# riveSunder/therldaisyworld

Measured on AMD Instinct MI355X. Metric: cell-updates/sec (grid x batch), fused stencil+growth step, higher is better.
Workload: dtype f32

## Files before the change

therldaisyworld_amd/csrc/dw_api.hip:

```cpp
#include <hip/hip_runtime.h>

#include <cmath>
#include <cstdarg>
#include <cstdio>
#include <cstdlib>
#include <cstring>
#include <memory>
#include <new>
#include <type_traits>
#include <vector>

#include "../../include/daisyworld_hip.h"
#include "dw_kernels.hpp"
#include "dw_host_util.hpp"
#include "dw_plan.hpp"
#include "dw_series.hpp"

using namespace dw;

static thread_local char g_err[512] = "";

static int fail(int code, const char* fmt, ...) {
    va_list ap;
    va_start(ap, fmt);
// ... 436 lines not shown
        });
    } else {
        const int prec = p.precision == DW_PRECISION_F64 ? 2 : (ex ? 0 : 1);
        with_int<2, 0, 1>(prec, [&](auto PR) { generic(iL, iD, PR); });
    }
    HIPCHK(hipGetLastError());
    step_done(h, 0.0, true, true, constants);
    return DW_OK;
}

static int launch_forward_fused2_pw(dw_handle* h, const PairPw* row, StatsDev* trace) {
    const StepPlan& pl = h->plan;
    const StepOut o = step_out(h);
    const FusedGeom& g = pl.fgeom;
    const dim3 grid((unsigned)g.chunk * 8u);
    const plane_t *inL = h->L16[h->cur].get(), *inD = h->D16[h->cur].get();
    with_int<kFusedRot, kFusedOvl>(pl.fused_mode, [&](auto MODE) {
        hipLaunchKernelGGL((trace_pair_fast_pw<MODE>), grid, dim3(256), 0, h->stream, inL, inD, o.L, o.D, g, row, o.zero_me,
                           o.zero_n, trace);
    });
    HIPCHK(hipGetLastError());
    step_done(h, 0.0, false, true, true);
    return DW_OK;
}

static int temp_chunks(const dw_handle* h) {
    return (int)(((long long)h->prm.height * h->prm.width + kTempChunk - 1) / kTempChunk);
}
static size_t temp_part_bytes(const dw_handle* h) { return sizeof(TempPartial) * (size_t)h->prm.batch * temp_chunks(h); }

static int launch_temp_moments(dw_handle* h, bool current, double L, const PhysF64* row64, TempStatsDev* out) {
    const dw_params& p = h->prm;
    const int chunks = temp_chunks(h);
    const PhysF64 P = row64 ? PhysF64{} : make_f64(p, L);
    TempPartial* part = h->temp_part.get();
    auto reduce = [&](auto* iL, auto* iD) {
        with_bool(row64 != nullptr, [&](auto TABLE) {
            hipLaunchKernelGGL((temp_moments_pw<elem_t<decltype(iL)>, TABLE>), dim3((unsigned)chunks, (unsigned)p.batch), dim3(256),
                               0, h->stream, iL, iD, p.height, p.width, P, row64, part);
        });
    };
    if (current) with_planes(h, h->unq == OWN_CUR, h->cur, reduce);
    else with_derived_from(h, [&](auto* iL, auto* iD, auto) { reduce(iL, iD); });
    HIPCHK(hipGetLastError());
    hipLaunchKernelGGL(temp_moments_finish_pw, dim3((unsigned)((p.batch + 63) / 64)), dim3(64), 0, h->stream, part, p.batch, chunks,
                       (double)p.height * (double)p.width, out);
    HIPCHK(hipGetLastError());
    return DW_OK;
}

template <class F>
static auto with_fused_layout(const StepPlan& pl, F&& f) {
    if (pl.packed) return f(int_c<kFusedRot>{}, std::true_type{});
    return with_int<kFusedRot, kFusedRing, kFusedOvl>(pl.fused_mode, [&](auto MODE) { return f(MODE, std::false_type{}); });
}

static int launch_forward_fused2(dw_handle* h, double L1, double L2, unsigned int* pstats = nullptr,
                                 float thr_hi = 0.f, StatsDev* trace = nullptr) {
    const dw_params& p = h->prm;
    const StepPlan& pl = h->plan;
    const bool exact = p.precision == DW_PRECISION_EXACT;
    PhysF32 P1, P2;
    if (exact) derive_f32_pair(p, L1, L2, &P1, &P2);
    else { P1 = derive_f32(p, L1); P2 = derive_f32(p, L2); }
    const StepOut o = step_out(h);
    const FusedGeom& g = pl.fgeom;
    const dim3 grid((unsigned)g.chunk * 8u);
    const plane_t *inL = h->L16[h->cur].get(), *inD = h->D16[h->cur].get();
    auto exact_args = [&] {
        return FusedExactArgs{inL, inD, o.L, o.D, g, P1, lum_part(P2), o.zero_me, o.zero_n, pstats, thr_hi, make_f64(p, L1), L1, L2};
    };
    if (trace && exact) {
        const TraceExactArgs A{exact_args(), trace, h->sw.force_rescan ? 1 : 0};
        with_int<kFusedRot, kFusedOvl>(pl.fused_mode, [&](auto MODE) {
            with_bool(pl.sym_albedo, [&](auto SYM) {
                hipLaunchKernelGGL((trace_pair_exact<MODE, SYM>), grid, dim3(256), 0, h->stream, A);
            });
        });
    } else if (trace) {
        with_int<kFusedRot, kFusedOvl>(pl.fused_mode, [&](auto MODE) {
            hipLaunchKernelGGL((trace_pair_fast<MODE>), grid, dim3(256), 0, h->stream, inL, inD, o.L, o.D, g, P1, P2, o.zero_me,
                               o.zero_n, trace);
        });
    } else if (pl.fmt_planes && !pstats && !exact) {
        hipLaunchKernelGGL((step_stream_fused2_fmt_pw<kFusedOvl>), grid, dim3(256), 0, h->stream, inL, inD, o.L, o.D, g, P1, P2,
                           o.zero_me, o.zero_n);
    } else if (exact) {
        const FusedExactArgs A = exact_args();
        with_bool(pstats != nullptr, [&](auto STATS) {
            with_fused_layout(pl, [&](auto MODE, auto PACK) {
                with_bool(pl.sym_albedo, [&](auto SYM) {
                    hipLaunchKernelGGL((step_stream_fused2_exact<MODE, PACK, STATS, SYM>), grid, dim3(256), 0, h->stream, A);
                });
            });
        });
    } else {
        with_bool(pstats != nullptr, [&](auto STATS) {
            with_fused_layout(pl, [&](auto MODE, auto PACK) {
                hipLaunchKernelGGL((step_stream_fused2<MODE, PACK, STATS>), grid, dim3(256), 0, h->stream, inL, inD, o.L, o.D, g,
                                   P1, P2, o.zero_me, o.zero_n, pstats, thr_hi);
            });
        });
    }
    HIPCHK(hipGetLastError());
    step_done(h, L2, false);
    return DW_OK;
}

static int launch_agents(dw_handle* h, const int* d_action, int act_b, int act_n, bool standalone = false,
                         double* d_reward = nullptr, unsigned char* d_done = nullptr, unsigned char* d_ok = nullptr) {
    const dw_params& p = h->prm;
    if (p.n_agents == 0) return DW_OK;
    NEED(h->have_state, DW_ESTATE, "no state uploaded");
    NEED(h->have_agents, DW_ESTATE, "no agents uploaded (call dw_upload_agents or dw_init_random)");
    NEED(p.collision_mode == 0 || standalone, DW_EINVAL,
         "collision_mode=1: call dw_update_agents, apply the collision pass (it consumes the caller's RNG) to the "
         "downloaded agent states, upload them, then dw_step without actions");
    const int blocks = (p.batch + 63) / 64;
    with_planes(h, h->unq == OWN_CUR, h->cur, [&](auto* L, auto* D) {
        using T = elem_t<decltype(L)>;
        hipLaunchKernelGGL(agents_update<T>, dim3(blocks), dim3(64), 0, h->stream, L, D, h->idx.get(), h->st.get(), d_action,
                           act_b, act_n, p.batch, p.n_agents, p.height, p.width, p.agent_gamma,
                           p.collision_mode == 0 ? 1 : 0, d_reward, d_done, d_ok);
    });
    HIPCHK(hipGetLastError());
    return DW_OK;
}

static int stage_host_actions(dw_handle* h, const int32_t* action, int b, int n) {
    const dw_params& p = h->prm;
    NEED(b >= 0 && n >= 0 && b <= p.batch && n <= p.n_agents, DW_EINVAL,
         "action block %dx%d exceeds (B,N)=(%d,%d)", b, n, p.batch, p.n_agents);
    if ((size_t)b * n)
        HIPCHK(hipMemcpyAsync(h->action_tmp.get(), action, sizeof(int) * (size_t)b * n, hipMemcpyHostToDevice,
                              h->stream));
    return DW_OK;
}

static int clear_stats(dw_handle* h) {
    for (int i = 0; i < 2; ++i) HIPCHK(hipMemsetAsync(h->stats2[i].get(), 0, h->stats_bytes, h->stream));
    return DW_OK;
}

static void state_arrived(dw_handle* h, UnqOwner unq, UnqKind kind = UNQ_F64) {
    if (unq == OWN_CUR) h->unq_kind = kind;
    h->unq = unq;
    h->have_state = true;
    h->stepped = false;
    for (auto& sn : h->snap) sn.valid = false;
}

template <class T>
static auto init_random_into(dw_handle* h, uint64_t seed, T* L, T* D) {
    const dw_params& p = h->prm;
    if (int crc = clear_stats(h)) return crc;
    const int ncell = p.height * p.width;
    const dim3 g((unsigned)((ncell + kInitChunk - 1) / kInitChunk), (unsigned)p.batch);
    hipLaunchKernelGGL((init_random_cells<T>), g, dim3(256), 0, h->stream, L, D, ncell,
                       (long long)p.world_offset, (unsigned long long)seed, (float)p.light_proportion,
                       (float)p.dark_proportion, (float)p.initial_al, (float)p.initial_ad, h->stats2[h->sp].get());
    HIPCHK(hipGetLastError());
    if (p.n_agents) {
        const int bn = p.batch * p.n_agents;
        hipLaunchKernelGGL(init_random_agents, dim3((bn + 255) / 256), dim3(256), 0, h->stream, h->idx.get(), h->st.get(),
                           p.batch, p.n_agents, p.height, p.width, (long long)p.world_offset,
                           (unsigned long long)seed);
// ... 1555 lines not shown
        job(h->idx.get(), sn.idx.get(), sizeof(int) * 2 * bn);
        job(h->st.get(), sn.st.get(), sizeof(double) * bn);
    }
    if (sn.stepped && sn.unq != OWN_PREV) {
        job(h->L16[1 - h->cur].get(), sn.PL.get(), pb);
        job(h->D16[1 - h->cur].get(), sn.PD.get(), pb);
    }
    if (int rc = launch_copy_regions(h, J)) return rc;
    HIPCHK(hipMemsetAsync(h->stats2[1 - h->sp].get(), 0, h->stats_bytes, h->stream));
    h->unq = sn.unq;
    h->stepped = sn.stepped;
    h->L_last = sn.L_last;
    h->L_per_world = sn.L_per_world;
    h->P_per_world = sn.P_per_world;
    return DW_OK;
}

int dw_snapshot_save(dw_handle* h) { return dw_snapshot_save_slot(h, 0); }
int dw_snapshot_restore(dw_handle* h) { return dw_snapshot_restore_slot(h, 0); }


int dw_set_stream(dw_handle* h, void* hip_stream) {
    NEED(h, DW_EINVAL, "null handle");
    HIPCHK(hipSetDevice(h->prm.device));
    HIPCHK(hipStreamSynchronize(h->stream));
    if (h->own_stream) HIPCHK(hipStreamDestroy(h->stream));
    h->stream = reinterpret_cast<hipStream_t>(hip_stream);
    h->own_stream = false;
    return DW_OK;
}

int dw_sync(dw_handle* h) {
    NEED(h, DW_EINVAL, "null handle");
    HIPCHK(hipSetDevice(h->prm.device));
    HIPCHK(hipStreamSynchronize(h->stream));
    return DW_OK;
}

int dw_timer_start(dw_handle* h) {
    NEED(h, DW_EINVAL, "null handle");
    HIPCHK(hipSetDevice(h->prm.device));
    HIPCHK(hipEventRecord(h->ev0, h->stream));
    return DW_OK;
}

int dw_timer_stop(dw_handle* h, float* elapsed_ms) {
    NEED(h && elapsed_ms, DW_EINVAL, "null argument");
    HIPCHK(hipSetDevice(h->prm.device));
    HIPCHK(hipEventRecord(h->ev1, h->stream));
    HIPCHK(hipEventSynchronize(h->ev1));
    HIPCHK(hipEventElapsedTime(elapsed_ms, h->ev0, h->ev1));
    return DW_OK;
}

int dw_device_planes(dw_handle* h, int which, void** light, void** dark) {
    NEED(h && light && dark, DW_EINVAL, "null argument");
    NEED(which == DW_STATE_CURRENT || which == DW_STATE_PREVIOUS, DW_EINVAL, "bad state selector");
    const int buf = which == DW_STATE_CURRENT ? h->cur : 1 - h->cur;
    NEED(which != DW_STATE_CURRENT || cur_quantised(h), DW_ESTATE,
         "the current state is an un-quantised upload: it has no binary16 planes before the first step");
    *light = h->L16[buf].get();
    *dark = h->D16[buf].get();
    return DW_OK;
}

int dw_kernel_info(dw_handle* h, char* buf, size_t buflen) {
    NEED(h && buf && buflen, DW_EINVAL, "null argument");
    const dw_params& p = h->prm;
    const StepPlan& pl = h->plan;
    const char* prec = p.precision == DW_PRECISION_EXACT ? "exact" : (p.precision == DW_PRECISION_FAST ? "fast" : "f64");
    static const char* const halo_name[] = {"rotate", "dpp-old", "general", "packed"};
    if (pl.kind == STEP_STREAM) {
        const StripGeom& g = pl.sgeom;
        snprintf(buf, buflen,
                 "step_stream_%s<halo=%s> wave-strip=%dx256 cells, register window + DPP neighbours, %d-row blocks in "
                 "flight%s, %d strips, grid=%d x 256 threads (4 strips each), XCD-chunked",
                 prec, halo_name[pl.halo], g.SR,
                 p.precision == DW_PRECISION_EXACT ? DW_STREAM_RB_EXACT : DW_STREAM_RB_FAST,
                 p.precision == DW_PRECISION_EXACT ? ", in-wave float64 fix-up from an LDS queue" : "", g.nstrips,
                 g.chunk * 8);
        if (pl.allow_fuse) {
            const size_t n = std::strlen(buf);
            snprintf(buf + n, buflen - n, "; dw_step_n fuses step pairs (step_stream_fused2%s%s)",
                     p.precision == DW_PRECISION_EXACT ? "_exact" : "", pl.fmt_planes ? "_fmt_pw, format buffer accesses" : "");
        }
    } else if (pl.kind == STEP_TILED) {
        const int TR = (256 / pl.tcq) * pl.rpt;
        snprintf(buf, buflen,
                 "step_tiled<TCQ=%d,RPT=%d,%s> tile=%dx%d cells, %zu B LDS/workgroup, %d tiles, grid=%d x 256 threads, "
                 "XCD-chunked",
                 pl.tcq, pl.rpt, prec, TR, pl.tcq * 4, pl.tile_lds, pl.geom.ntiles, pl.geom.chunk * 8);
    } else {
        snprintf(buf, buflen, "step_generic<%s> one thread per cell, grid=(%d,%d) x 256 threads", prec,
                 (p.height * p.width + 255) / 256, p.batch);
    }
    {
        const size_t n = std::strlen(buf);
        snprintf(buf + n, buflen - n, pl.trace_pairs ? "; trace: step pairs" : "; trace: single steps");
    }
    {
        const size_t n = std::strlen(buf);
        snprintf(buf + n, buflen - n, pl.pw_stream ? "; per-world L: wave strips" : "; per-world L: generic");
    }
    {
        static const char* const form_name[] = {"launches per step", "workgroup (LDS)", "one wave per world"};
        const size_t n = std::strlen(buf);
        snprintf(buf + n, buflen - n, "; episode: %s; mlp episode: %s", form_name[episode_form(h)], form_name[episode_mlp_form(h)]);
    }
    {
        const size_t n = std::strlen(buf);
        snprintf(buf + n, buflen - n, "; ensemble episode: %s", ensemble_episode_wave(h) ? "one wave per world" : "launches per step");
    }
    if (pl.first_stream) {
        const size_t n = std::strlen(buf);
        snprintf(buf + n, buflen - n, "; first step: wave-strip=%dx256", pl.first_geom.SR);
    }
    if (h->sw.text[0]) {
        const size_t n = std::strlen(buf);
        snprintf(buf + n, buflen - n, "; switches[%s]", h->sw.text);
    }
    {
        const size_t n = std::strlen(buf);
        snprintf(buf + n, buflen - n, "; per-world constants: %s",
                 ensemble_pairs(h) ? "step pairs" : (pl.pw_stream ? "wave strips" : "generic"));
    }
    return DW_OK;
}

int dw_audit_tie_bound(dw_handle* h, double L, double out[4]) {
    NEED(h && out, DW_EINVAL, "null argument");
    const dw_params& p = h->prm;
    HIPCHK(hipSetDevice(p.device));
    NEED(h->have_state && cur_quantised(h), DW_ESTATE, "the audit needs a quantised current state");
    const StepPlan& pl = h->plan;
    int rc = ensure_scratch(h, 4 * sizeof(unsigned long long));
    if (rc) return rc;
    unsigned long long* d = reinterpret_cast<unsigned long long*>(h->scratch.get());
    HIPCHK(hipMemsetAsync(d, 0, 4 * sizeof(unsigned long long), h->stream));
    const dim3 g((unsigned)((p.height * p.width + 255) / 256), (unsigned)p.batch);
    hipLaunchKernelGGL(tie_audit, g, dim3(256), 0, h->stream, h->L16[h->cur].get(), h->D16[h->cur].get(), p.height, p.width,
                       derive_f32(p, L), make_f64(p, L), d, pl.sym_albedo && pl.kind == STEP_STREAM ? 1 : 0);
    HIPCHK(hipGetLastError());
    unsigned long long r[4];
    HIPCHK(hipMemcpyAsync(r, d, sizeof(r), hipMemcpyDeviceToHost, h->stream));
    HIPCHK(hipStreamSynchronize(h->stream));
    std::memcpy(&out[0], &r[0], sizeof(double));
    std::memcpy(&out[1], &r[1], sizeof(double));
    out[2] = (double)r[2];
    out[3] = (double)r[3];
    return DW_OK;
}

int dw_last_fixup_count(dw_handle* h, uint64_t* count) {
    NEED(h && count, DW_EINVAL, "null argument");
    HIPCHK(hipSetDevice(h->prm.device));
    std::vector<StatsDev> st((size_t)h->prm.batch + 1);
    HIPCHK(hipMemcpyAsync(st.data(), h->stats2[h->sp].get(), sizeof(StatsDev) * st.size(), hipMemcpyDeviceToHost, h->stream));
    HIPCHK(hipStreamSynchronize(h->stream));
    unsigned long long v = st[h->prm.batch].sum_l;
    for (int b = 0; b < h->prm.batch; ++b) v += st[b].reserved;
    *count = v;
    return DW_OK;
}

}
```

therldaisyworld_amd/csrc/dw_kernels.hpp:

```cpp
#pragma once
#include "dw_common.hpp"
#include "dw_step_generic.hpp"
#include "dw_step_tiled.hpp"
#include "dw_step_stream.hpp"
#include "dw_step_fused.hpp"
#include "dw_step_first.hpp"
#include "dw_step_per_world.hpp"
#include "dw_step_fused_pw.hpp"
#include "dw_episode.hpp"
#include "dw_episode_wave.hpp"
#include "dw_agents.hpp"
#include "dw_state_io.hpp"
#include "dw_agents_fused.hpp"
#include "dw_temp_moments.hpp"
#include "dw_episode_wave_pw.hpp"
```

therldaisyworld_amd/csrc/dw_plan.hpp:

```cpp
#pragma once
#include <climits>
#include <cmath>
#include <cstddef>
#include <cstdio>
#include <cstdlib>
#include <cstring>

#include "../../include/daisyworld_hip.h"
#include "dw_types.hpp"

namespace dw {

struct Switches {
    bool no_sym = false, no_pack = false, no_fuse = false, no_ring = false, no_fmt_planes = false, no_episode_kernel = false,
         no_episode_wave = false, no_agent_fuse = false, no_agent_preapply = false, first_f64 = false,
         first_generic = false, force_rescan = false, test_hooks = false;
    int pack_min_strips = -1, strip_rows = 0, tile_rpt = 0, queue_cap = -1, mismatch_cap = -1, trace_rows = 0;
    double first_slack = -1.0;
    char kernel[16] = {0};
    char text[256] = {0};
};
inline const char* test_hook(const char* name) {
    return std::getenv("DW_TEST_HOOKS") ? std::getenv(name) : nullptr;
}
inline Switches read_switches() {
    Switches w;
    auto note = [&](const char* name, const char* val) {
        const size_t n = std::strlen(w.text);
        snprintf(w.text + n, sizeof(w.text) - n, "%s%s%s%s", n ? " " : "", name, val ? "=" : "", val ? val : "");
    };
    auto flag = [&](const char* name, bool& dst) { if (std::getenv(name)) { dst = true; note(name, nullptr); } };
    auto num = [&](const char* name, int& dst, bool test) {
        if (const char* e = test ? test_hook(name) : std::getenv(name)) { dst = std::atoi(e); note(name, e); }
    };
    w.test_hooks = std::getenv("DW_TEST_HOOKS") != nullptr;
    flag("DW_NO_SYM", w.no_sym); flag("DW_NO_PACK", w.no_pack); flag("DW_NO_FUSE", w.no_fuse); flag("DW_NO_RING", w.no_ring);
    flag("DW_NO_FMT_PLANES", w.no_fmt_planes);
    flag("DW_NO_EPISODE_KERNEL", w.no_episode_kernel); flag("DW_NO_EPISODE_WAVE", w.no_episode_wave);
    flag("DW_NO_AGENT_FUSE", w.no_agent_fuse); flag("DW_NO_AGENT_PREAPPLY", w.no_agent_preapply);
    flag("DW_FIRST_STEP_F64", w.first_f64); flag("DW_FIRST_GENERIC", w.first_generic);
    num("DW_PACK_MIN_STRIPS", w.pack_min_strips, false); num("DW_STRIP_ROWS", w.strip_rows, false);
    num("DW_TILE_RPT", w.tile_rpt, false);
    num("DW_TEST_QUEUE_CAP", w.queue_cap, true); num("DW_TEST_MISMATCH_CAP", w.mismatch_cap, true);
    num("DW_TEST_TRACE_ROWS", w.trace_rows, true);
    if (test_hook("DW_TEST_FORCE_RESCAN")) { w.force_rescan = true; note("DW_TEST_FORCE_RESCAN", nullptr); }
    if (const char* e = test_hook("DW_TEST_FIRST_SLACK")) { w.first_slack = std::atof(e); note("DW_TEST_FIRST_SLACK", e); }
    if (const char* e = std::getenv("DW_KERNEL")) { snprintf(w.kernel, sizeof(w.kernel), "%s", e); note("DW_KERNEL", e); }
    return w;
}

inline dw_params with_world_params(dw_params p, const dw_world_params& w) {
    p.p = w.p; p.g = w.g; p.S = w.S; p.sigma = w.sigma; p.gamma = w.gamma; p.q = w.q; p.q2 = w.q2; p.dt = w.dt;
    p.albedo_bare = w.albedo_bare; p.albedo_light = w.albedo_light; p.albedo_dark = w.albedo_dark;
    p.temp_optimal = w.temp_optimal;
    return p;
}
inline dw_world_params world_params_of(const dw_params& p) {
    return dw_world_params{p.p, p.g, p.S, p.sigma, p.gamma, p.q, p.q2, p.dt, p.albedo_bare, p.albedo_light, p.albedo_dark,
                           p.temp_optimal};
}
inline bool albedo_symmetric(double bare, double light, double dark) { return (dark - bare) == -(light - bare); }
inline bool worlds_symmetric(const dw_world_params* worlds, size_t B) {
    for (size_t b = 0; b < B; ++b)
        if (!albedo_symmetric(worlds[b].albedo_bare, worlds[b].albedo_light, worlds[b].albedo_dark)) return false;
    return true;
}

inline PhysF64 make_f64(const dw_params& p, double L) {
    PhysF64 P;
    P.p = p.p; P.g = p.g; P.S = p.S; P.sigma = p.sigma; P.gamma = p.gamma; P.q = p.q; P.q2 = p.q2;
    P.dt = p.dt; P.ab = p.albedo_bare; P.al = p.albedo_light; P.ad = p.albedo_dark;
    P.To = p.temp_optimal; P.L = L;
    const double e1 = std::exp(-1.0), e2 = std::exp(-2.0);
    const double s = 1.0 + 4.0 * e1 + 4.0 * e2;
    P.w0 = 1.0 / s; P.w1 = e1 / s; P.w2 = e2 / s;
    return P;
}

inline double cbeta_host(const dw_params& p) {
    const double cbeta = p.g * p.temp_optimal * p.temp_optimal;
    return cbeta > 1e-30 ? 1.0 / std::sqrt(cbeta) : 0x1p60;
}

inline void split_hi_lo(double v, double scale, float* hi, float* lo) {
    const double h = std::nearbyint(v * scale) / scale;
    *hi = (float)h;
    *lo = (float)(v - h);
}

inline float round_up(double v) {
    const float f = (float)v;
    return (double)f < v ? std::nextafterf(f, INFINITY) : f;
}

struct EConst { double c0l, c0d; };
inline EConst e_const(const dw_params& p, double L) {
    const double To4 = std::pow(p.temp_optimal, 4), K = p.S * L / p.sigma;
    const double e0 = K * (1.0 - p.albedo_bare * p.p) / To4 - 1.0;
    return EConst{e0 + p.q2 * (p.albedo_bare * p.p - p.albedo_light) / To4,
                  e0 + p.q2 * (p.albedo_bare * p.p - p.albedo_dark) / To4};
}

struct TieChain {
    double emin, emax, vlo;
    bool admissible;
    double ew;
    double kbmax;
    double pu, safety;
};
inline TieChain tie_chain(const dw_params& p, const EConst& c, double a1, double a2, double a3, double a4, double de) {
    const double u = std::ldexp(1.0, -24), kmax = 1000.0;
    TieChain t;
    const double pos = (std::fmax(a1, 0.0) + std::fmax(a2, 0.0)) * 8 * kmax + (std::fmax(a3, 0.0) + std::fmax(a4, 0.0)) * kmax;
    const double neg = (std::fmin(a1, 0.0) + std::fmin(a2, 0.0)) * 8 * kmax + (std::fmin(a3, 0.0) + std::fmin(a4, 0.0)) * kmax;
    t.emax = std::fmax(c.c0l, c.c0d) + pos;
    t.emin = std::fmin(c.c0l, c.c0d) + neg;
    const double vmin = 1.0 + t.emin, vmax = 1.0 + t.emax;
    t.admissible = vmin > 0.02;
    t.vlo = std::fmax(vmin, 0.02);
    const double smax = std::sqrt(std::fmax(vmax, t.vlo));
// ... 39 lines not shown
    P.a1 = (float)((double)P.a1h + P.a1l); P.a2 = (float)((double)P.a2h + P.a2l);
    P.a3 = (float)((double)P.a3h + P.a3l); P.a4 = (float)((double)P.a4h + P.a4l);
    P.c0ls = (float)((double)P.c0lh + P.c0ll); P.c0ds = (float)((double)P.c0dh + c0dl);
    const double kbe = cbeta_host(p);
    P.kbeta = (float)kbe;
    const PhysF64 P64 = make_f64(p, L);
    P.dw0 = (float)(p.dt * P64.w0); P.dw1 = (float)(p.dt * P64.w1); P.dw2 = (float)(p.dt * P64.w2);
    P.p = (float)p.p; P.ck = p.dt != 0.0 ? (float)(0.001 / p.dt) : 0.f;
    P.ngamma = (float)(-p.gamma);
    const double u = std::ldexp(1.0, -24);
    const double lo_mag = std::ldexp(1.0, -(hb + 1)) * 18.0 * kmax + std::ldexp(1.0, -(hb + 1));
    const double de_abs = 6.0 * u * lo_mag + 1e-9;
    const TieChain t = tie_chain(p, c0, a1, a2, a3, a4, de_abs);
    auto e_over_D2 = [&](double e) {
        const double v = std::fmax(1.0 + e, t.vlo), sv = std::sqrt(v), yv = std::sqrt(sv);
        const double D = kbe * (yv + 1.0) * (sv + 1.0);
        return std::fabs(e) / (D * D);
    };
    const double Ae = 2.0 * de_abs * std::fmax(e_over_D2(t.emin), e_over_D2(t.emax));
    double A0 = t.safety * (kmax * std::fabs(p.dt) * t.kbmax * Ae + 2e-6);
    if (!t.admissible) A0 = 1.0;
    const double eA = t.safety * 13.0 * u;
    const double eK0d = t.safety * (6.0 * std::fabs(p.p) + t.pu + t.kbmax + 8.0 * std::fabs(p.gamma)) * u;
    const double eK1d = t.safety * ((6.0 * std::fabs(p.p) + t.pu) * u + t.kbmax * (u + 2.0 * t.ew));
    P.tie_lo = (float)(0.5 - A0);
    if ((double)P.tie_lo > 0.5 - A0) P.tie_lo = std::nextafterf(P.tie_lo, -INFINITY);
    P.eA = round_up(eA);
    const float eK0 = round_up(eK0d), eK1 = round_up(eK1d);
    P.eK0s = p.dt < 0.0 ? eK0 : -eK0;
    P.eK1s = p.dt < 0.0 ? eK1 : -eK1;
    P.neK1s = -P.eK1s;
    P.eK01s = (float)((double)P.eK0s + (double)P.eK1s);
    if (std::fabs((double)P.eK01s) < std::fabs((double)P.eK0s + (double)P.eK1s))
        P.eK01s = std::nextafterf(P.eK01s, P.eK01s < 0.f ? -1.f : 1.f);
    return P;
}

inline void derive_f32_pair(const dw_params& p, double L1, double L2, PhysF32* P1, PhysF32* P2) {
    const PhysF32 a = derive_f32(p, L1), b = derive_f32(p, L2);
    const int hb = a.hi_bits < b.hi_bits ? a.hi_bits : b.hi_bits;
    *P1 = derive_f32(p, L1, hb);
    *P2 = derive_f32(p, L2, hb);
    const float tie_lo = P1->tie_lo < P2->tie_lo ? P1->tie_lo : P2->tie_lo;
    P1->tie_lo = tie_lo;
    P2->tie_lo = tie_lo;
}

inline FirstStepBound derive_first_bound(const dw_params& p, double L, const PhysF32& P, bool from_f64,
                                         double test_slack = -1.0) {
    const double u = std::ldexp(1.0, -24), iota = from_f64 ? u : 0.0;
    const double kmax = 1000.0;
    const double a1 = std::fabs((double)P.a1), a2 = std::fabs((double)P.a2), a3 = std::fabs((double)P.a3), a4 = std::fabs((double)P.a4);
    const EConst c0 = e_const(p, L);
    const double c0m = std::fmax(std::fabs(c0.c0l), std::fabs(c0.c0d));
    const double Mmax = (a1 + a2) * 8 * kmax + (a3 + a4) * kmax;
    const double de_max = (8.0 * u + iota) * Mmax + u * c0m;
    const TieChain t = tie_chain(p, c0, P.a1, P.a2, P.a3, P.a4, de_max);
    const double kbe = cbeta_host(p);
    const double Dmin = kbe * (std::sqrt(std::sqrt(t.vlo)) + 1.0) * (std::sqrt(t.vlo) + 1.0);
    const double kK = 5.0 * u + iota;
    const double safety = t.safety, pu = t.pu, kbmax = t.kbmax;
    FirstStepBound B;
    B.a1 = round_up(a1); B.a2 = round_up(a2); B.a3 = round_up(a3); B.a4 = round_up(a4);
    B.c_de = round_up(safety * (8.0 * u + iota) * (1.0 + 8.0 * u));
    B.c_c0 = round_up(safety * u * c0m);
    B.eK0 = round_up(safety * (pu + (kK + 2.0 * u) * std::fabs(p.p) + kbmax * u + ((kK + 3.0 * u) + u) * std::fabs(p.gamma)));
    B.eK1 = round_up(safety * (pu + (kK + 2.0 * u) * std::fabs(p.p) + kbmax * (u + 2.0 * t.ew)));
    B.cW = round_up(safety * 2.0 * kbmax / Dmin);
    B.eA = round_up(safety * ((kK + 3.0 * u) + u + (kK + u)));
    B.cS = round_up(safety * u);
    B.slack = t.admissible ? 4e-6f : 1.0f;
    if (test_slack > (double)B.slack) B.slack = (float)test_slack;
    return B;
}

enum StepKind { STEP_GENERIC, STEP_TILED, STEP_STREAM };
struct StepPlan {
    StepKind kind = STEP_GENERIC;
    int halo = 0;
    bool packed = false;
    bool allow_fuse = false;
    int fused_mode = kFusedOvl;
    bool fmt_planes = false;
    bool trace_pairs = false;
    bool sym_albedo = false;
    int tcq = 0, rpt = 0;
    Geom geom{};
    size_t tile_lds = 0;
    StripGeom sgeom{};
    FusedGeom fgeom{};
    int first_prec = 2;
    bool first_stream = false;
    FirstGeom first_geom{};
    bool need_fixq = false;
    bool pw_stream = false;
};

inline int halo_form(int W) { return W < 256 ? 3 : (W == 256 ? 0 : (W % 256 == 0 ? 1 : 2)); }

inline int strip_rows(long groups, int H, long target) {
    int sr = 64;
    while (sr > 8 && groups * ((H + sr - 1) / sr) < target) sr >>= 1;
    return H < sr ? H : sr;
}

inline int strip_rows_or_override(const Switches& sw, int cap, long groups, int H, long target) {
    if (sw.strip_rows < 1) return strip_rows(groups, H, target);
    const int want = sw.strip_rows < cap ? sw.strip_rows : cap;
    return H < want ? H : want;
}

inline StepPlan plan_steps(const dw_params& p, const Switches& sw) {
    StepPlan s;
    s.sym_albedo = albedo_symmetric(p.albedo_bare, p.albedo_light, p.albedo_dark) && !sw.no_sym;
    s.halo = halo_form(p.width);
    const int lpw = p.width / 4, wpr = lpw ? 64 / lpw : 0;
    const bool pack_shape = p.width >= 8 && p.width < 256 && wpr >= 1 && wpr * lpw * 10 >= 64 * 7 && !sw.no_pack;
    const long pack_strips = pack_shape ? (long)((p.batch + wpr - 1) / wpr) * ((p.height + 63) / 64) : 0;
    const bool packable = pack_shape && pack_strips >= (sw.pack_min_strips >= 0 ? sw.pack_min_strips : 512);
    const bool quads = p.precision != DW_PRECISION_F64 && p.width % 4 == 0;
    if (quads && (p.width >= 256 || packable) && std::strcmp(sw.kernel, "tiled") != 0) {
        s.kind = STEP_STREAM;
        s.packed = p.width < 256;
        StripGeom& g = s.sgeom;
        g.B = p.batch; g.H = p.height; g.W = p.width;
        g.ncs = (p.width + 255) / 256;
        g.lpw = s.packed ? lpw : 64;
        g.wpr = s.packed ? wpr : 1;
        const long groups = s.packed ? (p.batch + wpr - 1) / wpr : p.batch;
        g.SR = strip_rows_or_override(sw, INT_MAX, groups * g.ncs, p.height, 2048);
        g.nrs = (p.height + g.SR - 1) / g.SR;
        g.nstrips = (int)(groups * g.nrs * g.ncs);
        g.nwg = (g.nstrips + 3) / 4;
        g.chunk = (g.nwg + 7) / 8;
        g.qcap = kWaveQueueCap;
        int mcap = kMismatchCap;
        if (sw.queue_cap >= 0 && sw.queue_cap < kWaveQueueCap) g.qcap = sw.queue_cap;
        if (sw.mismatch_cap >= 0 && sw.mismatch_cap < kMismatchCap) mcap = sw.mismatch_cap;
        g.force_rescan = sw.force_rescan ? 1 : 0;
        s.allow_fuse = !sw.no_fuse;
        const bool ring = p.width == 1024 && !sw.no_ring;
        s.fused_mode = p.width <= 256 ? kFusedRot : (ring ? kFusedRing : kFusedOvl);
        FusedGeom& f = s.fgeom;
        f.B = p.batch; f.H = p.height; f.W = p.width;
        f.SR = g.SR;
        f.nrs = g.nrs;
        f.lpw = g.lpw; f.wpr = g.wpr;
        f.cols_per_strip = p.width <= 256 ? 256 : (ring ? 1024 : 248);
        f.ncs = s.packed ? 1 : (p.width + f.cols_per_strip - 1) / f.cols_per_strip;
        f.nstrips = (int)(groups * f.nrs * f.ncs);
        f.nwg = ring ? f.nstrips : (f.nstrips + 3) / 4;
        f.chunk = (f.nwg + 7) / 8;
        f.qcap = g.qcap;
        f.mcap = mcap;
        f.sure_need = 9 * p.n_agents + 9 * mcap + 1;
        s.trace_pairs = s.allow_fuse && !s.packed && s.fused_mode != kFusedRing;
        s.fmt_planes = p.precision == DW_PRECISION_FAST && s.allow_fuse && !s.packed && s.fused_mode == kFusedOvl && !sw.no_fmt_planes &&
                       (size_t)p.height * p.width * sizeof(plane_t) < ((size_t)1 << 31);
    } else if (quads && p.width >= 64) {
        s.kind = STEP_TILED;
        const int Wq = p.width / 4;
        if (Wq >= 64) {
            s.tcq = 64; s.rpt = 4;
            if (sw.tile_rpt == 2 || sw.tile_rpt == 4 || sw.tile_rpt == 8) s.rpt = sw.tile_rpt;
        }
        else if (Wq >= 32) { s.tcq = 32; s.rpt = 4; }
        else { s.tcq = 16; s.rpt = 2; }
        const int TR = (256 / s.tcq) * s.rpt;
        Geom& g = s.geom;
        g.B = p.batch; g.H = p.height; g.W = p.width; g.Wq = Wq;
        g.tiles_r = (p.height + TR - 1) / TR;
        g.tiles_c = (Wq + s.tcq - 1) / s.tcq;
        g.ntiles = p.batch * g.tiles_r * g.tiles_c;
        g.chunk = (g.ntiles + 7) / 8;
        g.qcap = kMaxFix;
        if (sw.queue_cap >= 0 && sw.queue_cap < kMaxFix) g.qcap = sw.queue_cap;
        s.tile_lds = (size_t)2 * (TR + 2) * (s.tcq + 2) * 4 * sizeof(float);
    }
    s.need_fixq = p.precision == DW_PRECISION_EXACT && s.kind == STEP_TILED;
    s.pw_stream = s.kind == STEP_STREAM && !s.packed;
    s.first_prec = p.precision == DW_PRECISION_FAST ? 1 : (p.precision == DW_PRECISION_EXACT && !sw.first_f64 ? 3 : 2);
    s.first_stream = (p.width % 256 == 0 || s.kind == STEP_STREAM) && s.first_prec != 2 && !sw.first_generic;
    if (s.first_stream) {
        FirstGeom& fg = s.first_geom;
        fg.B = p.batch; fg.H = p.height; fg.W = p.width;
        fg.lpw = s.packed ? lpw : 64;
        fg.wpr = s.packed ? wpr : 1;
        fg.ncs = s.packed ? 1 : (p.width + 255) / 256;
        const long groups = s.packed ? (p.batch + fg.wpr - 1) / fg.wpr : p.batch;
        fg.SR = strip_rows_or_override(sw, 64, groups * fg.ncs, p.height, 4096);
        fg.nrs = (p.height + fg.SR - 1) / fg.SR;
        fg.nstrips = (int)(groups * fg.nrs * fg.ncs);
    }
    return s;
}

}
```

therldaisyworld_amd/csrc/dw_types.hpp:

```cpp
#pragma once

namespace dw {

typedef _Float16 plane_t;

struct PhysF64 {
    double p, g, S, sigma, gamma, q, q2, dt;
    double ab, al, ad, To;
    double L;
    double w0, w1, w2;
};

typedef float dw_f32x2 __attribute__((ext_vector_type(2)));
#define DW_PAIR(lo_name, hi_name, pair_name) \
    union { struct { float lo_name, hi_name; }; dw_f32x2 pair_name; }

struct PhysF32 {
    DW_PAIR(a1h, a2h, a12h);
    DW_PAIR(a3h, a4h, a34h);
    DW_PAIR(a1l, a2l, a12l);
    DW_PAIR(a3l, a4l, a34l);
    DW_PAIR(c0lh, c0ll, c0l);
    DW_PAIR(c0dh, dc0l, c0d);
    DW_PAIR(a1, a2, a12);
    DW_PAIR(a3, a4, a34);
    DW_PAIR(c0ls, c0ds, c0s);
    DW_PAIR(dw0, dw1, dw01);
    DW_PAIR(dw2, kbeta, dw2kb);
    DW_PAIR(p, ck, pck);
    DW_PAIR(eK1s, eK0s, eKs);
    DW_PAIR(ngamma, tie_lo, gt);
    DW_PAIR(neK1s, eK01s, eKb);
    float eA;
    int hi_bits;
};
static_assert(sizeof(PhysF32) == 32 * sizeof(float), "PhysF32 layout");

struct PhysLumF32 {
    dw_f32x2 a12h, a12l, c0l, c0d, a12, c0s;
};

struct FirstStepBound {
    float a1, a2, a3, a4;
    float c_de, c_c0;
    float eK0, eK1, cW, eA, cS, slack;
};

struct PairPw {
    PhysF32 P1, P2;
};
static_assert(sizeof(PairPw) == 2 * sizeof(PhysF32), "PairPw layout");

struct StatsDev {
    unsigned int max_k;
    unsigned int reserved;
    unsigned long long sum_l;
    unsigned long long sum_d;
};

struct Geom {
    int B, H, W;
    int Wq;
    int tiles_r, tiles_c;
    int ntiles;
    int chunk;
    int qcap;
};

struct StripGeom {
    int B, H, W;
    int SR;
    int ncs, nrs;
    int nstrips;
    int nwg;
    int chunk;
    int qcap;
    int lpw, wpr;
    int force_rescan;
};

struct FusedGeom {
    int B, H, W;
    int SR;
    int ncs, nrs;
    int nstrips, nwg, chunk;
    int cols_per_strip;
    int qcap, mcap;
    int lpw, wpr;
    int sure_need;
};

struct FirstGeom {
    int B, H, W;
    int SR;
    int ncs, nrs;
    int nstrips;
    int lpw, wpr;
};

enum { kFusedOvl = 0, kFusedRot = 1, kFusedRing = 2 };
constexpr int kWaveQueueCap = 256;
constexpr int kMismatchCap = 64;
constexpr int kMaxFix = 1024;
constexpr int kNumQueues = 256;

}
```

Before: 820.1 billion.

## Add fused two-step kernel using full 256-column strips with LDS halo exchange

Adds a new fused step-pair kernel for widths that are multiples of 256. Each wave owns a full 256-column strip with no overlapping columns. The first-step edge columns are precomputed per strip and stored in LDS tables. Intermediate left and right neighbours are then exchanged through per-wave LDS slots rather than recomputed from overlapping halo columns. This removes redundant halo computation from the old 248-column overlapped strips, at the cost of LDS traffic, wave barriers, a scalar prologue recomputing the boundary columns, and inline exec-mask assembly.

```diff
diff --git a/therldaisyworld_amd/csrc/dw_api.hip b/therldaisyworld_amd/csrc/dw_api.hip
--- a/therldaisyworld_amd/csrc/dw_api.hip
+++ b/therldaisyworld_amd/csrc/dw_api.hip
@@ -542,6 +542,10 @@
             hipLaunchKernelGGL((trace_pair_fast<MODE>), grid, dim3(256), 0, h->stream, inL, inD, o.L, o.D, g, P1, P2, o.zero_me,
                                o.zero_n, trace);
         });
+    } else if (pl.full_strips && !pstats && !exact) {
+        const FusedGeom& q = pl.fullgeom;
+        hipLaunchKernelGGL(step_stream_fused2_full_pw, dim3((unsigned)q.chunk * 8u), dim3(256), 0, h->stream, inL, inD, o.L, o.D, q,
+                           P1, P2, o.zero_me, o.zero_n);
     } else if (pl.fmt_planes && !pstats && !exact) {
         hipLaunchKernelGGL((step_stream_fused2_fmt_pw<kFusedOvl>), grid, dim3(256), 0, h->stream, inL, inD, o.L, o.D, g, P1, P2,
                            o.zero_me, o.zero_n);
@@ -2263,7 +2267,8 @@
         if (pl.allow_fuse) {
             const size_t n = std::strlen(buf);
             snprintf(buf + n, buflen - n, "; dw_step_n fuses step pairs (step_stream_fused2%s%s)",
-                     p.precision == DW_PRECISION_EXACT ? "_exact" : "", pl.fmt_planes ? "_fmt_pw, format buffer accesses" : "");
+                     p.precision == DW_PRECISION_EXACT ? "_exact" : "", pl.full_strips ? "_full_pw, format buffer accesses, full 256-column strips"
+                                      : (pl.fmt_planes ? "_fmt_pw, format buffer accesses" : ""));
         }
     } else if (pl.kind == STEP_TILED) {
         const int TR = (256 / pl.tcq) * pl.rpt;
diff --git a/therldaisyworld_amd/csrc/dw_kernels.hpp b/therldaisyworld_amd/csrc/dw_kernels.hpp
--- a/therldaisyworld_amd/csrc/dw_kernels.hpp
+++ b/therldaisyworld_amd/csrc/dw_kernels.hpp
@@ -4,6 +4,7 @@
 #include "dw_step_tiled.hpp"
 #include "dw_step_stream.hpp"
 #include "dw_step_fused.hpp"
+#include "dw_step_fused_full.hpp"
 #include "dw_step_first.hpp"
 #include "dw_step_per_world.hpp"
 #include "dw_step_fused_pw.hpp"
diff --git a/therldaisyworld_amd/csrc/dw_plan.hpp b/therldaisyworld_amd/csrc/dw_plan.hpp
--- a/therldaisyworld_amd/csrc/dw_plan.hpp
+++ b/therldaisyworld_amd/csrc/dw_plan.hpp
@@ -12,7 +12,7 @@
 namespace dw {
 
 struct Switches {
-    bool no_sym = false, no_pack = false, no_fuse = false, no_ring = false, no_fmt_planes = false, no_episode_kernel = false,
+    bool no_sym = false, no_pack = false, no_fuse = false, no_ring = false, no_fmt_planes = false, no_full_strips = false, no_episode_kernel = false,
          no_episode_wave = false, no_agent_fuse = false, no_agent_preapply = false, first_f64 = false,
          first_generic = false, force_rescan = false, test_hooks = false;
     int pack_min_strips = -1, strip_rows = 0, tile_rpt = 0, queue_cap = -1, mismatch_cap = -1, trace_rows = 0;
@@ -35,7 +35,7 @@
     };
     w.test_hooks = std::getenv("DW_TEST_HOOKS") != nullptr;
     flag("DW_NO_SYM", w.no_sym); flag("DW_NO_PACK", w.no_pack); flag("DW_NO_FUSE", w.no_fuse); flag("DW_NO_RING", w.no_ring);
-    flag("DW_NO_FMT_PLANES", w.no_fmt_planes);
+    flag("DW_NO_FMT_PLANES", w.no_fmt_planes); flag("DW_NO_FULL_STRIPS", w.no_full_strips);
     flag("DW_NO_EPISODE_KERNEL", w.no_episode_kernel); flag("DW_NO_EPISODE_WAVE", w.no_episode_wave);
     flag("DW_NO_AGENT_FUSE", w.no_agent_fuse); flag("DW_NO_AGENT_PREAPPLY", w.no_agent_preapply);
     flag("DW_FIRST_STEP_F64", w.first_f64); flag("DW_FIRST_GENERIC", w.first_generic);
@@ -241,6 +241,8 @@
     bool allow_fuse = false;
     int fused_mode = kFusedOvl;
     bool fmt_planes = false;
+    bool full_strips = false;
+    FusedGeom fullgeom{};
     bool trace_pairs = false;
     bool sym_albedo = false;
     int tcq = 0, rpt = 0;
@@ -316,6 +318,21 @@
         s.trace_pairs = s.allow_fuse && !s.packed && s.fused_mode != kFusedRing;
         s.fmt_planes = p.precision == DW_PRECISION_FAST && s.allow_fuse && !s.packed && s.fused_mode == kFusedOvl && !sw.no_fmt_planes &&
                        (size_t)p.height * p.width * sizeof(plane_t) < ((size_t)1 << 31);
+        s.full_strips = s.fmt_planes && p.width % 256 == 0 && p.width >= 512 && !sw.no_full_strips;
+        if (s.full_strips) {
+            FusedGeom& q = s.fullgeom;
+            q = f;
+            q.cols_per_strip = 256;
+            q.ncs = p.width / 256;
+            q.SR = strip_rows_or_override(sw, kFullMaxRows, groups * q.ncs, p.height, 2048);
+            if (sw.strip_rows < 1 && q.SR == 64 && p.height > 64 &&
+                groups * q.ncs * ((p.height + kFullTallRows - 1) / kFullTallRows) >= 2048)
+                q.SR = p.height < kFullTallRows ? p.height : kFullTallRows;
+            q.nrs = (p.height + q.SR - 1) / q.SR;
+            q.nstrips = (int)(groups * q.nrs * q.ncs);
+            q.nwg = (q.nstrips + 3) / 4;
+            q.chunk = (q.nwg + 7) / 8;
+        }
     } else if (quads && p.width >= 64) {
         s.kind = STEP_TILED;
         const int Wq = p.width / 4;
diff --git a/therldaisyworld_amd/csrc/dw_step_fused_full.hpp b/therldaisyworld_amd/csrc/dw_step_fused_full.hpp
--- /dev/null
+++ b/therldaisyworld_amd/csrc/dw_step_fused_full.hpp
@@ -0,0 +1,207 @@
+#pragma once
+#include "dw_step_fused.hpp"
+
+#ifndef DW_FULL_DBG
+#define DW_FULL_DBG 0
+#endif
+namespace dw {
+
+constexpr int kFullTblBytes = ((kFullMaxRows + 4) / 3 + 1) * 8;
+constexpr int kFullSlotBytes = 64 * 16 + 2 * kFullTblBytes;
+constexpr int kFullWaveBytes = 3 * kFullSlotBytes;
+
+typedef __attribute__((address_space(3))) unsigned char dw_lds_byte;
+typedef __attribute__((address_space(3))) dw_f32x2 dw_lds_f32x2;
+typedef __attribute__((address_space(3))) float dw_lds_f32;
+
+__device__ float dw_buf_load_fmt1(dw_i32x4 rsrc, int voff, int soff, int aux) __asm("llvm.amdgcn.raw.buffer.load.format.f32");
+__device__ __forceinline__ dw_i32x4 fmt_cell_rsrc(dw_i32x4 plane_rsrc) {
+    plane_rsrc.w = 0x00017004;
+    return plane_rsrc;
+}
+
+__device__ __forceinline__ void fused2_full_body(const plane_t* __restrict__ inL, const plane_t* __restrict__ inD,
+                                                 plane_t* __restrict__ outL, plane_t* __restrict__ outD, const FusedGeom& G,
+                                                 const PhysF32& P1, const PhysF32& P2,
+                                                 unsigned long long* __restrict__ zero_me, int zero_n) {
+    __shared__ dw_fmt_f32x4 s_full[4 * kFullWaveBytes / 16];
+    const int bid = blockIdx.x;
+    const int wg = (bid & 7) * G.chunk + (bid >> 3);
+    if (wg >= G.nwg) return;
+    const int tid = threadIdx.x, wv = tid >> 6, lane = tid & 63;
+    if (wg == 0)
+        for (int i = tid; i < zero_n; i += 256) zero_me[i] = 0ull;
+    const int s = __builtin_amdgcn_readfirstlane(wg * 4 + wv);
+    if (s >= G.nstrips) return;
+    const int spw = G.nrs * G.ncs;
+    const int b = s / spw;
+    const int sw = s - b * spw;
+    const int rs = sw / G.ncs, cs = sw - rs * G.ncs;
+    const int r0 = rs * G.SR;
+    const int nr = min(G.SR, G.H - r0);
+    const int col = 256 * cs + 4 * lane;
+    const int c_left = cs == 0 ? G.W - 1 : 256 * cs - 1;
+    const int c_right = cs == G.ncs - 1 ? 0 : 256 * cs + 256;
+
+    const unsigned int world_bytes = (unsigned int)(G.H * G.W) * 2u;
+    const dw_i32x4 fmt_inL = fmt_plane_rsrc(inL, b, world_bytes), fmt_inD = fmt_plane_rsrc(inD, b, world_bytes);
+    const dw_i32x4 fmt_outL = fmt_plane_rsrc(outL, b, world_bytes), fmt_outD = fmt_plane_rsrc(outD, b, world_bytes);
+    const dw_i32x4 cell_inL = fmt_cell_rsrc(fmt_inL), cell_inD = fmt_cell_rsrc(fmt_inD);
+    const int fmt_col = col * 2, fmt_row = G.W * 2;
+    const int fmt_lnb = (lane == 0 ? c_left : col - 1) * 2, fmt_rnb = (lane == 63 ? c_right : col + 4) * 2;
+
+    dw_lds_byte* const lds = (dw_lds_byte*)s_full + wv * kFullWaveBytes;
+
+    {
+        const plane_t* pL = inL + (size_t)b * G.H * G.W;
+        const plane_t* pD = inD + (size_t)b * G.H * G.W;
+        auto column = [&](int c, int tbl) {
+#pragma clang fp contract(off)
+            const int cols[3] = {c == 0 ? G.W - 1 : c - 1, c, c == G.W - 1 ? 0 : c + 1};
+            for (int j = 1 + lane; j <= nr + 2; j += 64) {
+                const int rm = wrap_near(r0 - 2 + j, G.H);
+                const int rows[3] = {rm == 0 ? G.H - 1 : rm - 1, rm, rm == G.H - 1 ? 0 : rm + 1};
+                float l[3][3], d[3][3];
+#pragma unroll
+                for (int x = 0; x < 3; ++x)
+#pragma unroll
+                    for (int y = 0; y < 3; ++y) {
+                        const size_t o = (size_t)rows[x] * G.W + cols[y];
+                        l[x][y] = (float)pL[o];
+                        d[x][y] = (float)pD[o];
+                    }
+                const float El = (l[1][0] + l[1][2]) + (l[0][1] + l[2][1]), Cl = (l[0][0] + l[0][2]) + (l[2][0] + l[2][2]);
+                const float Ed = (d[1][0] + d[1][2]) + (d[0][1] + d[2][1]), Cd = (d[0][0] + d[0][2]) + (d[2][0] + d[2][2]);
+                const GrowthT<float> g = growth_t<kFastSplit, float>(P1, l[1][1], d[1][1], El, Cl, Ed, Cd);
+                const dw_f32x2 v{finish_fast(l[1][1], g.dKl, g.fl), finish_fast(d[1][1], g.dKd, g.fd)};
+                *(dw_lds_f32x2*)(lds + (j % 3) * kFullSlotBytes + tbl + ((j - 1) / 3) * 8) = v;
+            }
+        };
+        column(c_left, 1024);
+        column(c_right, 1024 + kFullTblBytes);
+    }
+    dw_lds_byte* lds_put = lds + 16 * lane;
+    dw_lds_byte* lds_lnb = lds + (lane == 0 ? 1024 : 16 * (lane - 1));
+    dw_lds_byte* lds_rnb = lds + (lane == 63 ? 1024 + kFullTblBytes : 16 * (lane + 1) + 8);
+    asm volatile("" : "+v"(lds_put), "+v"(lds_lnb), "+v"(lds_rnb));
+    __builtin_amdgcn_fence(__ATOMIC_RELEASE, "wavefront");
+    __builtin_amdgcn_wave_barrier();
+    __builtin_amdgcn_fence(__ATOMIC_ACQUIRE, "wavefront");
+
+    struct RawFull { float4 l, d; float la, lc, da, dc; };
+    auto row_offset = [&](int rr) -> int {
+        rr = min(rr, r0 + nr + 1);
+        rr = rr < 0 ? rr + G.H : rr;
+        rr = rr >= G.H ? rr - G.H : rr;
+        return rr * fmt_row;
+    };
+    auto load_cells = [&](int so, RawFull& w) {
+        w.l = fmt_load4(fmt_inL, fmt_col, so);
+        w.d = fmt_load4(fmt_inD, fmt_col, so);
+    };
+    auto load_nbrs = [&](int so, RawFull& w) {
+        w.la = dw_buf_load_fmt1(cell_inL, fmt_lnb, so, 0);
+        w.lc = dw_buf_load_fmt1(cell_inL, fmt_rnb, so, 0);
+        w.da = dw_buf_load_fmt1(cell_inD, fmt_lnb, so, 0);
+        w.dc = dw_buf_load_fmt1(cell_inD, fmt_rnb, so, 0);
+    };
+    auto load_raw = [&](int rr) -> RawFull {
+        RawFull w;
+        load_cells(row_offset(rr), w);
+        load_nbrs(row_offset(rr), w);
+        return w;
+    };
+    auto input_rows = [&](const RawFull& w, Row4& L, Row4& D) {
+        L = make_row(widen4(w.l), w.la, w.lc);
+        D = make_row(widen4(w.d), w.da, w.dc);
+    };
+
+    Row4 IL[3], ID[3], SL[3], SD[3];
+    input_rows(load_raw(r0 - 2), IL[0], ID[0]);
+    input_rows(load_raw(r0 - 1), IL[1], ID[1]);
+    input_rows(load_raw(r0), IL[2], ID[2]);
+    auto iter = [&](auto U, auto D1, auto D2, int j) {
+        constexpr int u = decltype(U)::value;
+        constexpr bool do1 = decltype(D1)::value, do2 = decltype(D2)::value;
+        RawFull nx;
+        const int nx_off = do1 ? row_offset(r0 + j) : 0;
+        if (do1) load_cells(nx_off, nx);
+#if DW_FULL_DBG == 2
+        if (do1) load_nbrs(nx_off, nx);
+#endif
+        __builtin_amdgcn_sched_barrier(0);
+        float l1[4], d1[4], l2[4], d2[4];
+        bool* const no_tie = nullptr;
+        if (do2)
+            cells4<false, false, bool>(P2, SL[u], SL[(u + 1) % 3], SL[(u + 2) % 3], SD[u], SD[(u + 1) % 3], SD[(u + 2) % 3], l2, d2, no_tie);
+        if (DW_FULL_DBG == 2) {
+        } else if (do1 && do2) {
+            __builtin_amdgcn_sched_barrier(0);
+            load_nbrs(nx_off, nx);
+            __builtin_amdgcn_sched_barrier(0);
+        } else if (do1) {
+            load_nbrs(nx_off, nx);
+        }
+        if (do1)
+            cells4<false, false, bool>(P1, IL[(u + 2) % 3], IL[u], IL[(u + 1) % 3], ID[(u + 2) % 3], ID[u], ID[(u + 1) % 3], l1, d1, no_tie);
+#if DW_FULL_DBG == 3
+        if (do1) __builtin_amdgcn_s_waitcnt(0);
+#endif
+        if (do2 && j <= nr + 3) {
+            fmt_store4(fmt_outL, fmt_col, (r0 + j - 4) * fmt_row, make_float4(l2[0], l2[1], l2[2], l2[3]));
+            fmt_store4(fmt_outD, fmt_col, (r0 + j - 4) * fmt_row, make_float4(d2[0], d2[1], d2[2], d2[3]));
+        }
+        if (do1) {
+            {
+                dw_lds_f32* const put = (dw_lds_f32*)(lds_put + u * kFullSlotBytes);
+                put[0] = l1[3]; put[1] = d1[3]; put[2] = l1[0]; put[3] = d1[0];
+            }
+            __builtin_amdgcn_fence(__ATOMIC_RELEASE, "wavefront");
+            __builtin_amdgcn_wave_barrier();
+            __builtin_amdgcn_fence(__ATOMIC_ACQUIRE, "wavefront");
+            const dw_f32x2 nb_l = *(const dw_lds_f32x2*)(lds_lnb + u * kFullSlotBytes);
+            const dw_f32x2 nb_r = *(const dw_lds_f32x2*)(lds_rnb + u * kFullSlotBytes);
+            __builtin_amdgcn_sched_barrier(0);
+            input_rows(nx, IL[(u + 2) % 3], ID[(u + 2) % 3]);
+            __builtin_amdgcn_sched_barrier(0);
+            SL[u] = make_row(make_float4(l1[0], l1[1], l1[2], l1[3]), nb_l.x, nb_r.x);
+            SD[u] = make_row(make_float4(d1[0], d1[1], d1[2], d1[3]), nb_l.y, nb_r.y);
+        }
+    };
+    using U0 = std::integral_constant<int, 0>;
+    using U1 = std::integral_constant<int, 1>;
+    using U2 = std::integral_constant<int, 2>;
+    using Yes = std::true_type;
+    using No = std::false_type;
+    auto next_trip = [&] {
+#if DW_FULL_DBG == 1
+        lds_lnb += (lane == 0 ? 8 : 0); lds_rnb += (lane == 63 ? 8 : 0);
+        return;
+#endif
+        asm volatile("s_mov_b64 exec, 1\n\t"
+                     "v_add_u32_e32 %0, 8, %0\n\t"
+                     "s_lshl_b64 exec, 1, 63\n\t"
+                     "v_add_u32_e32 %1, 8, %1\n\t"
+                     "s_mov_b64 exec, -1"
+                     : "+v"(lds_lnb), "+v"(lds_rnb) : : "scc");
+    };
+    iter(U1{}, Yes{}, No{}, 1);
+    iter(U2{}, Yes{}, No{}, 2);
+    iter(U0{}, Yes{}, No{}, 3);
+    next_trip();
+    for (int j = 4; j <= nr + 3; j += 3) {
+        iter(U1{}, Yes{}, Yes{}, j);
+        iter(U2{}, Yes{}, Yes{}, j + 1);
+        iter(U0{}, Yes{}, Yes{}, j + 2);
+        next_trip();
+    }
+}
+
+__global__ __launch_bounds__(256) __attribute__((amdgpu_waves_per_eu(DW_FUSED_FAST_WAVES, DW_FUSED_FAST_WAVES)))
+void step_stream_fused2_full_pw(const plane_t* __restrict__ inL, const plane_t* __restrict__ inD,
+                                plane_t* __restrict__ outL, plane_t* __restrict__ outD, FusedGeom G, PhysF32 P1, PhysF32 P2,
+                                unsigned long long* __restrict__ zero_me, int zero_n) {
+    fused2_full_body(inL, inD, outL, outD, G, P1, P2, zero_me, zero_n);
+}
+
+}
diff --git a/therldaisyworld_amd/csrc/dw_types.hpp b/therldaisyworld_amd/csrc/dw_types.hpp
--- a/therldaisyworld_amd/csrc/dw_types.hpp
+++ b/therldaisyworld_amd/csrc/dw_types.hpp
@@ -98,6 +98,8 @@
     int lpw, wpr;
 };
 
+constexpr int kFullMaxRows = 128;
+constexpr int kFullTallRows = 126;
 enum { kFusedOvl = 0, kFusedRot = 1, kFusedRing = 2 };
 constexpr int kWaveQueueCap = 256;
 constexpr int kMismatchCap = 64;
```

Result: slower. 701.8 billion (-14.4%).
